# RustAudio/lewton

Measured on NVIDIA H100. Metric: Msamples/s IMDCT+window+OLA, 2048-pt long blocks, higher is better.
Workload: dtype f32

## Files before the change

lewton_b200/build.py:

```python
import os
import re
import shutil
import subprocess

HERE = os.path.dirname(os.path.abspath(__file__))
CSRC = os.path.join(HERE, "csrc")
SO = os.path.join(HERE, "liblewton_b200.so")
K_LONG_REGS = 249
SOURCES = ["lwb_api.cu", "host_objects.cuh", "path_generic.cuh", "path_long.cuh", "path_chain.cuh", "path_mixed.cuh", "path_mid.cuh",
           "tables_host.cpp", "frontend.cpp", "lwb_common.h", "pcm_copy_plan.h", "kernels_generic.cuh", "kernel_long.cuh", "kernel_deal.cuh", "kernel_short.cuh", "kernel_mid.cuh", "kernel_chain.cuh", "kernel_prologue.cuh", "kernel_floor0.cuh", "floor1_eval.cuh",
           "floor1_inverse_db.inc", "Makefile"]


def _stale():
    if not os.path.exists(SO):
        return True
    t = os.path.getmtime(SO)
    deps = [os.path.join(CSRC, s) for s in SOURCES] + [os.path.join(HERE, "..", "include", h)
                                                       for h in ("lewton_b200.h", "lewton_frontend.h")]
    return any(os.path.getmtime(d) > t for d in deps)


def check_no_fma(so=SO):
    if shutil.which("cuobjdump") is None:
        return None
    sass = subprocess.run(["cuobjdump", "-sass", so], capture_output=True, text=True, check=True).stdout
    bad = re.findall(r"^\s+/\*[0-9a-f]+\*/\s+(?:@!?U?P[0-9T]\s+)?(FFMA2?|DFMA)\b.*$", sass, re.M)
    return len(bad)


def hot_kernel_registers(log):
    regs = {}
    for m in re.finditer(r"Compiling entry function '(_ZN3lwb6k_longI([fs])EE[^']*)'.*?Used (\d+) registers", log, re.S):
        regs["k_long<float>" if m.group(2) == "f" else "k_long<int16_t>"] = int(m.group(3))
    return regs


def build(force=False, verbose=False):
    if force or _stale():
        if shutil.which("nvcc") is None:
            raise RuntimeError("nvcc not found: lewton_b200 has no CPU fallback and cannot be built without CUDA")
# ... 21 lines not shown
```

lewton_b200/csrc/kernel_long.cuh:

```cuda
#pragma once
#include <stdint.h>

#if defined(__CUDACC__)
#include <cuda_runtime.h>
#define LWB_HD __host__ __device__ __forceinline__
#else
#define LWB_HD inline
#endif

namespace lwb {

constexpr int kLongBs = 11;
constexpr int kLongN = 2048;
constexpr int kLongN2 = 1024;

struct alignas(16) LongRun {
    const float *in;
    void *out;
    float *state;
    uint32_t in_stride;
    uint32_t n_packets;
    uint8_t has_prev;
    uint8_t write_state;
    uint8_t dummy;
// ... 322 lines not shown
            const V b2 = vadd(O[b][d], O[b][e]);
            const V b3 = vsub(E[b][d], E[b][e]);
            O[b][d] = vadd(b2, b0);
            E[b][d] = vadd(b3, b1);
            O[b][e] = vsub(b2, b0);
            E[b][e] = vsub(b1, b3);
        }
    }
}

LWB_HD void step8_ola(V b0, V b1, V wlo, V whi, V Oj, V Ej, V prev_lo, V prev_hi, V &pcm_lo, V &pcm_hi, V &p_even)
{
    const V p_odd = vsub_p(vmul(Oj, b1), vmul(Ej, b0));
    p_even = vnsub_p(vmul(Oj, b0), vmul(Ej, b1));
    pcm_lo = vadd_p(vmul(p_odd, wlo), vmul(prev_lo, whi));
    pcm_hi = vsub_p(vmul(prev_hi, wlo), vmul(p_odd, whi));
}

#if defined(__CUDACC__)
#ifndef LWB_LONG_NB
#define LWB_LONG_NB 1
#endif
#ifndef LWB_LONG_WARPS
#define LWB_LONG_WARPS 8
#endif
#ifndef LWB_LONG_RING
#define LWB_LONG_RING (LWB_LONG_NB == 2 ? 2 : 5)
#endif
constexpr int kLongNB = LWB_LONG_NB;
constexpr int kLongWarps = LWB_LONG_WARPS;
constexpr int kLongRing = LWB_LONG_RING;
constexpr int kLongTileBytes = kLongN2 * 4;
constexpr int kLongStageBytes = kLongNB * kLongTileBytes;
constexpr size_t kLongSmemBytes = 2048 + (size_t)kLongWarps * (kLongRing + 1) * kLongStageBytes +
                                  (size_t)kLongPackFloats * 4 + kLongWarps * (kLongRing + 2) * 8 +
                                  kLongWarps * kLongNB * sizeof(LongRun) + 64;

__device__ __forceinline__ uint32_t smem_u32(const void *p) { return (uint32_t)__cvta_generic_to_shared(p); }

__device__ __forceinline__ void mbar_init(uint32_t bar, uint32_t count)
{
    asm volatile("mbarrier.init.shared::cta.b64 [%0], %1;" ::"r"(bar), "r"(count));
}
__device__ __forceinline__ void mbar_expect_tx(uint32_t bar, uint32_t bytes)
{
    asm volatile("mbarrier.arrive.expect_tx.shared::cta.b64 _, [%0], %1;" ::"r"(bar), "r"(bytes) : "memory");
}
__device__ __forceinline__ void mbar_wait(uint32_t bar, uint32_t parity)
{
    asm volatile(
        "{\n\t.reg .pred p;\n\t"
        "WAIT_%=:\n\t"
        "mbarrier.try_wait.parity.shared::cta.b64 p, [%0], %1, %2;\n\t"
        "@p bra DONE_%=;\n\t"
        "bra WAIT_%=;\n\t"
        "DONE_%=:\n\t}" ::"r"(bar), "r"(parity), "r"(200000u) : "memory");
}
__device__ __forceinline__ void tma_load_1d(uint32_t dst, const void *src, uint32_t bytes, uint32_t bar)
{
    asm volatile("cp.async.bulk.shared::cluster.global.mbarrier::complete_tx::bytes [%0], [%1], %2, [%3];"
                 ::"r"(dst), "l"(src), "r"(bytes), "r"(bar) : "memory");
}
__device__ __forceinline__ void fence_proxy_async()
{
    asm volatile("fence.proxy.async.shared::cta;" ::: "memory");
}
__device__ __forceinline__ void sts_eo(uint32_t addr, float e, float o)
{
    asm volatile("st.shared.f32 [%0], %1;\n\tst.shared.f32 [%0+2048], %2;" ::"r"(addr), "f"(e), "f"(o) : "memory");
}
__device__ __forceinline__ void lds_eo(uint32_t addr, float &e, float &o)
{
    asm volatile("ld.shared.f32 %0, [%2];\n\tld.shared.f32 %1, [%2+2048];" : "=f"(e), "=f"(o) : "r"(addr) : "memory");
}

}
#include "kernel_deal.cuh"
namespace lwb {

#ifndef LWB_TW_REG0
#define LWB_TW_REG0 0
#endif
#ifndef LWB_TW_REG1
#define LWB_TW_REG1 (LWB_LONG_NB == 2 ? 0 : 53)
#endif
constexpr int kTwReg0 = LWB_TW_REG0;
constexpr int kTwReg1 = LWB_TW_REG1;
struct TwMix {
    const V *r;
    const V *lane_base;
    __device__ __forceinline__ V operator()(int slot) const
    {
        return (slot >= kTwReg0 && slot < kTwReg1) ? r[slot - kTwReg0] : lane_base[slot * 32];
    }
};
// ... 6 lines not shown
#define LWB_KC(j) (4u * (uint32_t)swz(j))

struct RunCur {
    const float *in;
    void *out;
    float *state;
    uint32_t in_stride;
    uint32_t flags;
};
__device__ __forceinline__ RunCur run_cur(const LongRun &r)
{
    return RunCur{r.in, r.out, r.state, r.in_stride,
                  (uint32_t)(r.has_prev ? 1u : 0u) | (r.write_state ? 2u : 0u) | (r.dummy ? 4u : 0u) |
                      (r.first_short ? 8u : 0u) | (r.last_short ? 16u : 0u)};
}
struct RunCurS : RunCur { float *state_out; };
__device__ __forceinline__ RunCurS run_cur_s(const LongRun &r)
{
    RunCurS c;
    static_cast<RunCur &>(c) = run_cur(r);
    c.flags |= r.first_short == 2 ? 32u : 0u;
    c.state_out = r.state_out ? r.state_out : r.state;
    return c;
}

__device__ __forceinline__ int16_t d_sample_i16(float v)
{
    short r;
    asm("cvt.rzi.s16.f32 %0, %1;" : "=h"(r) : "f"(__fmul_rn(v, 32768.0f)));
    return (int16_t)r;
}
__device__ __forceinline__ void st_pcm(float *p, float v) { __stcs(p, v); }
__device__ __forceinline__ void st_pcm(int16_t *p, float v) { __stcs(reinterpret_cast<short *>(p), (short)d_sample_i16(v)); }

template <int NB, bool FIRST, typename OutT, typename RC = RunCur>
__device__ __forceinline__ void out_stage(const TwMix &tw, int lane, const V O[NB][8], const V E[NB][8], V pe[NB][8],
                                          const RC cur[NB], OutT *out[NB], const float *s_state)
{
#pragma unroll
    for (int j = 0; j < 8; j++) {
        const int r64 = 64 * rev3(j);
        const bool nat = (j & 1);
        const V b0 = tw(P_B0 + j), b1 = tw(P_B1 + j);
        const V wlo = tw(P_WLO + j), whi = tw(P_WHI + j);
#pragma unroll
        for (int b = 0; b < NB; b++) {
            V plo = pe[b][j], phi = pe[b][j];
            bool emit = !(cur[b].flags & 4u);
            if (FIRST) {
                emit = emit && (cur[b].flags & 1u);
                if (cur[b].flags & 1u) {
                    const float *s_lo = s_state + b * kLongN2 + lane, *s_hi = s_state + b * kLongN2 + 63 - lane;
                    const float ax = nat ? s_lo[r64] : s_hi[r64], ay = nat ? s_hi[r64] : s_lo[r64];
                    const float bx = nat ? s_hi[960 - r64] : s_lo[960 - r64];
                    const float by = nat ? s_lo[960 - r64] : s_hi[960 - r64];
                    plo = V{ax, ay};
                    phi = V{bx, by};
                }
            }
            V lo, hi, pev;
            step8_ola(b0, b1, wlo, whi, O[b][j], E[b][j], plo, phi, lo, hi, pev);
            pe[b][j] = pev;
            if (emit) {
                OutT *o_lo = out[b] + lane, *o_hi = out[b] + 63 - lane;
                if (nat) {
                    st_pcm(o_lo + r64, lo.x); st_pcm(o_hi + r64, lo.y);
                    st_pcm(o_hi + 960 - r64, hi.x); st_pcm(o_lo + 960 - r64, hi.y);
                } else {
                    st_pcm(o_hi + r64, lo.x); st_pcm(o_lo + r64, lo.y);
                    st_pcm(o_lo + 960 - r64, hi.x); st_pcm(o_hi + 960 - r64, hi.y);
                }
            }
        }
    }
}

__device__ __forceinline__ float lds_f32(uint32_t addr)
{
    float v;
    asm volatile("ld.shared.f32 %0, [%1];" : "=f"(v) : "r"(addr) : "memory");
    return v;
}

template <int NB, typename OutT, typename RC = RunCur, bool EXPORT = false, int LS = 0>
__device__ __forceinline__ void out_first_short(const TwMix &tw, int lane, const V O[NB][8], const V E[NB][8], V pe[NB][8],
                                                const RC cur[NB], OutT *out[NB], const float *s_state,
                                                const float *__restrict__ w, int ls_arg, uint32_t w_s = 0)
{
    const int ls = LS ? LS : ls_arg;
    const int pl = kLongN2 - 2 * ls;
#pragma unroll
    for (int j = 0; j < 8; j++) {
        const int r64 = 64 * rev3(j);
        const bool nat = (j & 1);
        const V b0 = tw(P_B0 + j), b1 = tw(P_B1 + j);
#pragma unroll
// ... 9 lines not shown
                const int m = r64 + ((h == 0) == nat ? lane : 63 - lane);
                static_assert(LS % 64 == 0, "LS must be a multiple of 64");
                const bool on_slope = LS ? (r64 >= LS) : (m >= ls);
                if (on_slope) {
                    const int i = m - ls;
                    const float cw = __fmul_rn(po, (EXPORT ? lds_f32(w_s + 4u * (uint32_t)i) : __ldg(w + i)));
                    if (exported) cur[b].state[i] = cw;
                    else st_pcm(out[b] + i, __fadd_rn(cw, __fmul_rn(prev[i], (EXPORT ? lds_f32(w_s + 4u * (uint32_t)(pl - 1 - i)) : __ldg(w + pl - 1 - i)))));
                }
                const int i = kLongN2 - 1 - m - ls;
                float v = -po;
                if (LS ? on_slope : (i < pl)) {
                    v = __fmul_rn(v, (EXPORT ? lds_f32(w_s + 4u * (uint32_t)i) : __ldg(w + i)));
                    if (exported) { cur[b].state[i] = v; continue; }
                    v = __fadd_rn(v, __fmul_rn(prev[i], (EXPORT ? lds_f32(w_s + 4u * (uint32_t)(pl - 1 - i)) : __ldg(w + pl - 1 - i))));
                }
                st_pcm(out[b] + i, v);
            }
        }
    }
}

template <typename OutT>
__global__ void __launch_bounds__(kLongWarps * 32, 1)
k_long(const LongRun *__restrict__ runs, uint32_t n_groups, const float *__restrict__ pack,
       unsigned int *__restrict__ ticket, const float *__restrict__ w_short, int ls)
{
    constexpr int NB = kLongNB;
    extern __shared__ __align__(128) unsigned char smem_raw[];
    const int lane = threadIdx.x & 31, warp = threadIdx.x >> 5;
    const uint32_t raw_s = smem_u32(smem_raw);
    const uint32_t align_pad = (2048u - (raw_s & 2047u)) & 2047u;
    unsigned char *base = smem_raw + align_pad;
    constexpr size_t kTilesBytes = (size_t)kLongWarps * kLongRing * kLongStageBytes;
    constexpr size_t kStateBytes = (size_t)kLongWarps * kLongStageBytes;
    float *tiles = reinterpret_cast<float *>(base) + (size_t)warp * kLongRing * NB * kLongN2;
    float *s_state = reinterpret_cast<float *>(base + kTilesBytes) + (size_t)warp * NB * kLongN2;
    V *s_pack = reinterpret_cast<V *>(base + kTilesBytes + kStateBytes);
    unsigned char *tail = base + kTilesBytes + kStateBytes + (size_t)kLongPackFloats * 4;
    LongRun *s_next = reinterpret_cast<LongRun *>(tail) + warp * NB;
    uint64_t *bars = reinterpret_cast<uint64_t *>(tail + (size_t)kLongWarps * NB * sizeof(LongRun)) +
                     warp * (kLongRing + 2);
    if (n_groups == 0) return;

    {
        const float4 *src = reinterpret_cast<const float4 *>(pack);
        float4 *dst = reinterpret_cast<float4 *>(s_pack);
        for (int i = threadIdx.x; i < kLongPackFloats / 4; i += blockDim.x) dst[i] = __ldg(src + i);
    }
    if (lane == 0) {
        for (int i = 0; i < kLongRing + 2; i++) mbar_init(smem_u32(&bars[i]), 1);
        asm volatile("fence.mbarrier_init.release.cluster;" ::: "memory");
    }
    __syncthreads();

    V twR[kTwReg1 - kTwReg0 > 0 ? kTwReg1 - kTwReg0 : 1];
#pragma unroll
    for (int s = kTwReg0; s < kTwReg1; s++) twR[s - kTwReg0] = s_pack[s * 32 + lane];
    const TwMix tw{twR, s_pack + lane};

    const uint32_t tiles_s = smem_u32(tiles);
    const uint32_t bars_s = smem_u32(bars);
    const uint32_t bar_state = bars_s + 8 * kLongRing, bar_desc = bars_s + 8 * (kLongRing + 1);
    const uint32_t state_s = smem_u32(s_state), next_s = smem_u32(s_next);
    const uint32_t lA0 = laneA(lane, 0), lA1 = laneA(lane, 1);
    const uint32_t lB = laneB(lane);
    const uint32_t lC0 = laneC(lane, 0), lC1 = laneC(lane, 1);
    uint32_t phase_bits = 0;
    uint32_t slot_i = 0;

    uint32_t lc = 0;
    uint32_t nx_idx = 0;
    uint32_t nx_stage = 0;
    uint32_t nx_lc = 0, nx_npk = 0;
    uint32_t nx_state_issued = 0;
    uint32_t desc_parity = 0;
    RunCur cur[NB];
    uint32_t npk;

    auto issue_stage = [&](uint32_t stage, const LongRun *r, uint32_t pkt) {
        const uint32_t bar = bars_s + 8 * stage;
        mbar_expect_tx(bar, kLongStageBytes);
#pragma unroll
        for (int b = 0; b < NB; b++)
            tma_load_1d(tiles_s + stage * kLongStageBytes + b * kLongTileBytes,
                        r[b].in + (size_t)pkt * r[b].in_stride, kLongTileBytes, bar);
    };
    auto issue_stage_cur = [&](uint32_t stage, uint32_t pkt) {
        const uint32_t bar = bars_s + 8 * stage;
        mbar_expect_tx(bar, kLongStageBytes);
#pragma unroll
        for (int b = 0; b < NB; b++)
            tma_load_1d(tiles_s + stage * kLongStageBytes + b * kLongTileBytes,
                        cur[b].in + (size_t)pkt * cur[b].in_stride, kLongTileBytes, bar);
    };
    auto issue_state = [&](const float *const st[NB], const uint32_t has[NB]) {
        uint32_t bytes = 0;
#pragma unroll
        for (int b = 0; b < NB; b++) bytes += has[b] ? kLongTileBytes : 0;
        mbar_expect_tx(bar_state, bytes);
#pragma unroll
        for (int b = 0; b < NB; b++)
            if (has[b]) tma_load_1d(state_s + b * kLongTileBytes, st[b], kLongTileBytes, bar_state);
    };

    {
        uint32_t idx = 0;
        if (lane == 0) idx = atomicAdd(ticket, 1u);
        idx = __shfl_sync(0xffffffffu, idx, 0);
        if (idx >= n_groups) return;
#pragma unroll
        for (int b = 0; b < NB; b++) cur[b] = run_cur(runs[idx * NB + b]);
        npk = runs[idx * NB].n_packets;
        if (lane == 0) {
            fence_proxy_async();
            const float *st[NB];
            uint32_t has[NB];
#pragma unroll
            for (int b = 0; b < NB; b++) { st[b] = cur[b].state; has[b] = cur[b].flags & 1u; }
            issue_state(st, has);
            for (; lc < (uint32_t)kLongRing && lc < npk; lc++) issue_stage_cur(lc, lc);
            nx_idx = atomicAdd(ticket, 1u);
        }
    }

    for (;;) {
        V pe[NB][8];
#pragma unroll
        for (int b = 0; b < NB; b++)
#pragma unroll
            for (int j = 0; j < 8; j++) pe[b][j] = V{0.f, 0.f};
        OutT *out[NB];
#pragma unroll
        for (int b = 0; b < NB; b++) out[b] = static_cast<OutT *>(cur[b].out);

        for (uint32_t p = 0; p < npk; p++) {
            const uint32_t stage_s = tiles_s + slot_i * kLongStageBytes;
            mbar_wait(bars_s + 8 * slot_i, (phase_bits >> slot_i) & 1u);
            phase_bits ^= 1u << slot_i;

            V O[NB][8], E[NB][8];
            {
                const float *tp[NB];
#pragma unroll
                for (int b = 0; b < NB; b++) tp[b] = tiles + (slot_i * NB + b) * kLongN2;
                phase_a<NB>(tp, lane, tw, O, E);
            }
            __syncwarp();
#pragma unroll
            for (int b = 0; b < NB; b++) {
                const uint32_t t = stage_s + b * kLongTileBytes;
                const uint32_t a0 = t + lA0, a1 = t + lA1;
#pragma unroll
                for (int j = 0; j < 8; j++) {
// ... 16 lines not shown
#pragma unroll
            for (int b = 0; b < NB; b++) {
                const uint32_t b0 = stage_s + b * kLongTileBytes + lB;
#pragma unroll
                for (int j = 0; j < 8; j++) {
                    sts_eo(b0 ^ LWB_KB(j, 0), E[b][j].x, O[b][j].x);
                    sts_eo(b0 ^ LWB_KB(j, 1), E[b][j].y, O[b][j].y);
                }
            }
            __syncwarp();
#pragma unroll
            for (int b = 0; b < NB; b++) {
                const uint32_t t = stage_s + b * kLongTileBytes;
                const uint32_t c0 = t + lC0, c1 = t + lC1;
#pragma unroll
                for (int j = 0; j < 8; j++) {
                    lds_eo(c0 ^ LWB_KC(j), E[b][j].x, O[b][j].x);
                    lds_eo(c1 ^ LWB_KC(j), E[b][j].y, O[b][j].y);
                }
            }
            __syncwarp();
            if (lane == 0) {
                if (nx_stage == 0 && p >= 1) {
                    if (nx_idx < n_groups) {
                        fence_proxy_async();
                        mbar_expect_tx(bar_desc, NB * (uint32_t)sizeof(LongRun));
                        tma_load_1d(next_s, runs + (size_t)nx_idx * NB, NB * (uint32_t)sizeof(LongRun), bar_desc);
                        nx_stage = 1;
                    } else {
                        nx_stage = 3;
                    }
                }
                uint32_t ahead = lc - (p + 1) + nx_lc;
                if (ahead < (uint32_t)kLongRing) {
                    uint32_t tgt = slot_i + 1 + ahead;
                    if (tgt >= (uint32_t)kLongRing) tgt -= kLongRing;
                    if (lc < npk) {
                        fence_proxy_async();
                        issue_stage_cur(tgt, lc);
                        lc++;
                    } else {
                        if (nx_stage == 1) {
                            mbar_wait(bar_desc, desc_parity);
                            desc_parity ^= 1u;
                            nx_stage = 2;
                            nx_npk = s_next[0].n_packets;
                            nx_lc = 0;
                        }
                        if (nx_stage == 2 && nx_lc < nx_npk) {
                            fence_proxy_async();
                            issue_stage(tgt, s_next, nx_lc);
                            nx_lc++;
                        }
                    }
                }
            }
            phase_c_fft<NB>(tw, O, E);
            if (p > 0) {
                out_stage<NB, false, OutT>(tw, lane, O, E, pe, cur, out, s_state);
            } else {
                mbar_wait(bar_state, (phase_bits >> 30) & 1u);
                phase_bits ^= 1u << 30;
                if (NB == 1 && (cur[0].flags & 8u))
                    out_first_short<NB, OutT>(tw, lane, O, E, pe, cur, out, s_state, w_short, ls);
                else
                    out_stage<NB, true, OutT>(tw, lane, O, E, pe, cur, out, s_state);
                __syncwarp();
            }
#pragma unroll
            for (int b = 0; b < NB; b++)
                if (p > 0 || (cur[b].flags & 1u)) out[b] += (p == 0 && (cur[b].flags & 8u)) ? kLongN2 - ls : kLongN2;
            if (lane == 0 && nx_stage == 2 && !nx_state_issued) {
                const float *st[NB];
                uint32_t has[NB];
#pragma unroll
                for (int b = 0; b < NB; b++) { st[b] = s_next[b].state; has[b] = s_next[b].has_prev; }
                fence_proxy_async();
                issue_state(st, has);
                nx_state_issued = 1;
            }
            slot_i = (slot_i + 1 == (uint32_t)kLongRing) ? 0 : slot_i + 1;
        }
#pragma unroll
        for (int b = 0; b < NB; b++) {
            if ((cur[b].flags & 16u)) {
                const bool emitted = (npk > 1 || (cur[b].flags & 1u)) && !(cur[b].flags & 4u);
                const bool keep = (cur[b].flags & 6u) == 2u;
#pragma unroll
                for (int j = 0; j < 8; j++) {
                    const int r64 = 64 * rev3(j);
#pragma unroll
                    for (int h = 0; h < 2; h++) {
                        const float v = ((j & 1) != 0) == (h == 0) ? pe[b][j].x : pe[b][j].y;
                        const int m = r64 + (h ? 63 - lane : lane);
                        if (m < ls) {
                            if (emitted) st_pcm(out[b] + m, v);
                        } else if (keep && m < kLongN2 - ls) {
                            cur[b].state[m - ls] = v;
                            cur[b].state[kLongN2 - 1 - ls - m] = v;
                        }
                    }
                }
            } else if ((cur[b].flags & 6u) == 2u) {
                float *s_lo = cur[b].state + lane, *s_hi = cur[b].state + 63 - lane;
#pragma unroll
                for (int j = 0; j < 8; j++) {
                    const int r64 = 64 * rev3(j);
                    const float vx = (j & 1) ? pe[b][j].x : pe[b][j].y, vy = (j & 1) ? pe[b][j].y : pe[b][j].x;
                    s_lo[r64] = vx; s_hi[r64] = vy;
                    s_hi[960 - r64] = vx; s_lo[960 - r64] = vy;
                }
            }
        }
        uint32_t st_ = 0, nlc = 0;
        if (lane == 0) {
            if (nx_stage == 0) {
                if (nx_idx < n_groups) {
                    fence_proxy_async();
                    mbar_expect_tx(bar_desc, NB * (uint32_t)sizeof(LongRun));
                    tma_load_1d(next_s, runs + (size_t)nx_idx * NB, NB * (uint32_t)sizeof(LongRun), bar_desc);
                    nx_stage = 1;
                } else {
                    nx_stage = 3;
                }
            }
            if (nx_stage == 1) {
                mbar_wait(bar_desc, desc_parity);
                desc_parity ^= 1u;
                nx_stage = 2;
                nx_npk = s_next[0].n_packets;
                nx_lc = 0;
            }
            if (nx_stage == 2 && !nx_state_issued) {
                const float *st[NB];
                uint32_t has[NB];
#pragma unroll
                for (int b = 0; b < NB; b++) { st[b] = s_next[b].state; has[b] = s_next[b].has_prev; }
                fence_proxy_async();
                issue_state(st, has);
            }
            st_ = nx_stage;
            nlc = nx_lc;
        }
        st_ = __shfl_sync(0xffffffffu, st_, 0);
        nlc = __shfl_sync(0xffffffffu, nlc, 0);
        if (st_ != 2) break;
        __syncwarp();
#pragma unroll
        for (int b = 0; b < NB; b++) cur[b] = run_cur(s_next[b]);
        npk = s_next[0].n_packets;
        __syncwarp();
        lc = nlc;
        nx_stage = 0; nx_lc = 0; nx_npk = 0; nx_state_issued = 0;
        if (lane == 0) {
            fence_proxy_async();
            for (uint32_t k = lc; k < (uint32_t)kLongRing && k < npk; k++) {
                issue_stage_cur((slot_i + k) % kLongRing, k);
                lc = k + 1;
            }
            nx_idx = atomicAdd(ticket, 1u);
        }
    }
}

constexpr int kLongLs256 = (kLongN - 256) / 4;
constexpr int kLongFetch = 3;
constexpr int kLongDescSlots = kLongFetch + kLongRing + 3;
constexpr int kLongSlopeMax = 512;
constexpr size_t kLongSmemBytesS = 2048 + (size_t)kLongWarps * (kLongRing + 1) * kLongTileBytes + (size_t)kLongPackFloats * 4 +
                                   kLongWarps * (kLongRing + 2) * 8 + (size_t)kLongWarps * kLongDescSlots * sizeof(LongRun) +
                                   kLongSlopeMax * sizeof(float) + 64;

__device__ __forceinline__ void transpose_abc(const TwMix &tw, uint32_t stage_s, uint32_t lA0, uint32_t lA1, uint32_t lB,
                                              uint32_t lC0, uint32_t lC1, V O[1][8], V E[1][8])
{
    __syncwarp();
    {
        const uint32_t a0 = stage_s + lA0, a1 = stage_s + lA1;
#pragma unroll
        for (int j = 0; j < 8; j++) {
            sts_eo(a0 ^ LWB_KA(j), E[0][j].x, O[0][j].x);
            sts_eo(a1 ^ LWB_KA(j), E[0][j].y, O[0][j].y);
        }
    }
    __syncwarp();
    {
        const uint32_t b0 = stage_s + lB;
#pragma unroll
        for (int j = 0; j < 8; j++) {
            lds_eo(b0 ^ LWB_KB(j, 0), E[0][j].x, O[0][j].x);
            lds_eo(b0 ^ LWB_KB(j, 1), E[0][j].y, O[0][j].y);
        }
    }
    __syncwarp();
    phase_b<1>(tw, O, E);
// ... 195 lines not shown
```

profiles/microbench/io_skeleton.cu:

```cuda
#include <cuda_runtime.h>
#include <cstdio>
#include <cstdint>
#include <cstdlib>

__device__ __forceinline__ uint32_t smem_u32(const void *p) { return (uint32_t)__cvta_generic_to_shared(p); }
__device__ __forceinline__ void mbar_init(uint32_t bar, uint32_t c) { asm volatile("mbarrier.init.shared::cta.b64 [%0], %1;" ::"r"(bar), "r"(c)); }
__device__ __forceinline__ void mbar_expect_tx(uint32_t bar, uint32_t b) { asm volatile("mbarrier.arrive.expect_tx.shared::cta.b64 _, [%0], %1;" ::"r"(bar), "r"(b) : "memory"); }
__device__ __forceinline__ void mbar_wait(uint32_t bar, uint32_t parity)
{
    asm volatile("{\n\t.reg .pred p;\n\tW_%=:\n\tmbarrier.try_wait.parity.shared::cta.b64 p, [%0], %1;\n\t@p bra D_%=;\n\tbra W_%=;\n\tD_%=:\n\t}" ::"r"(bar), "r"(parity) : "memory");
}
__device__ __forceinline__ void tma_load_1d(uint32_t dst, const void *src, uint32_t bytes, uint32_t bar)
{
    asm volatile("cp.async.bulk.shared::cluster.global.mbarrier::complete_tx::bytes [%0], [%1], %2, [%3];" ::"r"(dst), "l"(src), "r"(bytes), "r"(bar) : "memory");
}

template <int MODE>
__global__ void __launch_bounds__(384, 1) k_io(const float *__restrict__ in, float *__restrict__ out, uint32_t n_chains,
                                               uint32_t packets, unsigned int *ticket)
{
    extern __shared__ __align__(128) unsigned char smem[];
    const int lane = threadIdx.x & 31, warp = threadIdx.x >> 5;
    float *tiles = reinterpret_cast<float *>(smem) + warp * 3 * 1024;
    uint64_t *bars = reinterpret_cast<uint64_t *>(smem + 12 * 3 * 4096) + warp * 3;
    if (lane == 0) { for (int i = 0; i < 3; i++) mbar_init(smem_u32(&bars[i]), 1); asm volatile("fence.mbarrier_init.release.cluster;" ::: "memory"); }
    __syncthreads();
    uint32_t phase = 0;
    for (;;) {
        uint32_t c = 0;
        if (lane == 0) c = atomicAdd(ticket, 1u);
        c = __shfl_sync(0xffffffffu, c, 0);
        if (c >= n_chains) break;
        const float *src = in + (size_t)(c >> 1) * packets * 2048 + (c & 1) * 1024;
        float *dst = out + (size_t)c * packets * 1024;
        if (lane == 0)
            for (uint32_t i = 0; i < 3 && i < packets; i++) {
                mbar_expect_tx(smem_u32(&bars[i]), 4096);
                tma_load_1d(smem_u32(tiles + i * 1024), src + (size_t)i * 2048, 4096, smem_u32(&bars[i]));
            }
        uint32_t s = 0;
        for (uint32_t p = 0; p < packets; p++) {
            mbar_wait(smem_u32(&bars[s]), (phase >> s) & 1u);
            phase ^= 1u << s;
            const float4 *t4 = reinterpret_cast<const float4 *>(tiles + s * 1024);
            float4 q[8];
#pragma unroll
            for (int m = 0; m < 4; m++) { q[m] = t4[lane + 64 * m]; q[4 + m] = t4[63 - lane + 64 * m]; }
            __syncwarp();
            if (lane == 0 && p + 3 < packets) {
                asm volatile("fence.proxy.async.shared::cta;" ::: "memory");
                mbar_expect_tx(smem_u32(&bars[s]), 4096);
                tma_load_1d(smem_u32(tiles + s * 1024), src + (size_t)(p + 3) * 2048, 4096, smem_u32(&bars[s]));
            }
            float *o = dst + (size_t)p * 1024;
            if (MODE == 0) {
                const float v[32] = {q[0].x, q[0].y, q[0].z, q[0].w, q[1].x, q[1].y, q[1].z, q[1].w, q[2].x, q[2].y, q[2].z, q[2].w,
                                     q[3].x, q[3].y, q[3].z, q[3].w, q[4].x, q[4].y, q[4].z, q[4].w, q[5].x, q[5].y, q[5].z, q[5].w,
                                     q[6].x, q[6].y, q[6].z, q[6].w, q[7].x, q[7].y, q[7].z, q[7].w};
#pragma unroll
                for (int j = 0; j < 8; j++) {
                    const int r64 = 64 * (((j & 1) << 2) | (j & 2) | ((j >> 2) & 1));
                    __stcs(o + lane + r64, v[4 * j]);
                    __stcs(o + 63 - lane + r64, v[4 * j + 1]);
                    __stcs(o + 63 - lane + 960 - r64, v[4 * j + 2]);
                    __stcs(o + lane + 960 - r64, v[4 * j + 3]);
                }
            } else {
                float4 *o4 = reinterpret_cast<float4 *>(o);
#pragma unroll
                for (int m = 0; m < 8; m++) __stcs(o4 + lane + 32 * m, q[m]);
            }
            s = (s + 1 == 3) ? 0 : s + 1;
        }
    }
}

int main(int argc, char **argv)
{
    const uint32_t streams = 4096, packets = 16, chains = streams * 2;
    const size_t n = (size_t)chains * packets * 1024;
    float *in, *out;
    unsigned int *ticket;
    cudaMalloc(&in, n * 4); cudaMalloc(&out, n * 4); cudaMalloc(&ticket, 4096);
    cudaMemset(in, 0, n * 4);
    const size_t smem = 12 * 3 * 4096 + 12 * 3 * 8 + 64;
    cudaFuncSetAttribute(k_io<0>, cudaFuncAttributeMaxDynamicSharedMemorySize, (int)smem);
    cudaFuncSetAttribute(k_io<1>, cudaFuncAttributeMaxDynamicSharedMemorySize, (int)smem);
    int sms = 0;
    cudaDeviceGetAttribute(&sms, cudaDevAttrMultiProcessorCount, 0);
    cudaEvent_t e0, e1; cudaEventCreate(&e0); cudaEventCreate(&e1);
    for (int mode = 0; mode < 2; mode++) {
        float best = 1e9f;
        for (int it = 0; it < 12; it++) {
            cudaMemset(ticket, 0, 4);
            cudaEventRecord(e0);
            if (mode == 0) k_io<0><<<sms, 384, smem>>>(in, out, chains, packets, ticket);
            else k_io<1><<<sms, 384, smem>>>(in, out, chains, packets, ticket);
            cudaEventRecord(e1); cudaEventSynchronize(e1);
            float ms; cudaEventElapsedTime(&ms, e0, e1);
            if (it >= 2 && ms < best) best = ms;
        }
        printf("mode %d (%s): best %.3f ms  -> %.1f GB/s (read+write), err=%s\n", mode, mode ? "STG.128 coalesced" : "k_long line order STG.32",
               best, 2.0 * n * 4 / best / 1e6, cudaGetErrorString(cudaGetLastError()));
    }
    float best = 1e9f;
    for (int it = 0; it < 8; it++) {
        cudaEventRecord(e0); cudaMemcpyAsync(out, in, n * 4, cudaMemcpyDeviceToDevice); cudaEventRecord(e1); cudaEventSynchronize(e1);
        float ms; cudaEventElapsedTime(&ms, e0, e1); if (it >= 2 && ms < best) best = ms;
    }
    printf("cudaMemcpy D2D: best %.3f ms -> %.1f GB/s\n", best, 2.0 * n * 4 / best / 1e6);
    return 0;
}
```

Baseline: 322,800.

## Stage k_long PCM and state output in shared memory and write via bulk async stores

Each warp now writes its output block to a shared-memory staging tile and issues a TMA bulk store (cp.async.bulk, evict_first hint for PCM) instead of scattered per-lane STG.32 streaming stores. The final state write-back goes through the same staging path. To free shared memory for the staging tiles, the input prefetch ring drops by one stage. This aims to cut the store instruction count and the uncoalesced write traffic, at the cost of a shallower load pipeline and extra bulk-group waits before each stage is reused.

Result: no change. 325,100 (median of 6 runs) (+0.7%).

```diff
diff --git a/lewton_b200/build.py b/lewton_b200/build.py
--- a/lewton_b200/build.py
+++ b/lewton_b200/build.py
@@ -6,7 +6,7 @@
 HERE = os.path.dirname(os.path.abspath(__file__))
 CSRC = os.path.join(HERE, "csrc")
 SO = os.path.join(HERE, "liblewton_b200.so")
-K_LONG_REGS = 249
+K_LONG_REGS = 244
 SOURCES = ["lwb_api.cu", "host_objects.cuh", "path_generic.cuh", "path_long.cuh", "path_chain.cuh", "path_mixed.cuh", "path_mid.cuh",
            "tables_host.cpp", "frontend.cpp", "lwb_common.h", "pcm_copy_plan.h", "kernels_generic.cuh", "kernel_long.cuh", "kernel_deal.cuh", "kernel_short.cuh", "kernel_mid.cuh", "kernel_chain.cuh", "kernel_prologue.cuh", "kernel_floor0.cuh", "floor1_eval.cuh",
            "floor1_inverse_db.inc", "Makefile"]
diff --git a/lewton_b200/csrc/kernel_long.cuh b/lewton_b200/csrc/kernel_long.cuh
--- a/lewton_b200/csrc/kernel_long.cuh
+++ b/lewton_b200/csrc/kernel_long.cuh
@@ -378,9 +378,11 @@
 constexpr int kLongRing = LWB_LONG_RING;
 constexpr int kLongTileBytes = kLongN2 * 4;
 constexpr int kLongStageBytes = kLongNB * kLongTileBytes;
-constexpr size_t kLongSmemBytes = 2048 + (size_t)kLongWarps * (kLongRing + 1) * kLongStageBytes +
-                                  (size_t)kLongPackFloats * 4 + kLongWarps * (kLongRing + 2) * 8 +
+constexpr int kLongRingK = kLongRing - 1;
+constexpr size_t kLongSmemBytes = 2048 + (size_t)kLongWarps * (kLongRingK + 2) * kLongStageBytes +
+                                  (size_t)kLongPackFloats * 4 + kLongWarps * (kLongRingK + 2) * 8 +
                                   kLongWarps * kLongNB * sizeof(LongRun) + 64;
+static_assert(kLongSmemBytes <= 227 * 1024, "k_long needs more than the 227 KB of shared memory a CTA can opt in to");
 
 __device__ __forceinline__ uint32_t smem_u32(const void *p) { return (uint32_t)__cvta_generic_to_shared(p); }
 
@@ -407,6 +409,20 @@
     asm volatile("cp.async.bulk.shared::cluster.global.mbarrier::complete_tx::bytes [%0], [%1], %2, [%3];"
                  ::"r"(dst), "l"(src), "r"(bytes), "r"(bar) : "memory");
 }
+__device__ __forceinline__ void bulk_store_1d(void *dst, uint32_t src, uint32_t bytes)
+{
+    asm volatile("cp.async.bulk.global.shared::cta.bulk_group [%0], [%1], %2;\n\tcp.async.bulk.commit_group;"
+                 ::"l"(dst), "r"(src), "r"(bytes) : "memory");
+}
+__device__ __forceinline__ void bulk_store_1d_stream(void *dst, uint32_t src, uint32_t bytes)
+{
+    asm volatile("{\n\t.reg .b64 pol;\n\t"
+                 "createpolicy.fractional.L2::evict_first.b64 pol, 1.0;\n\t"
+                 "cp.async.bulk.global.shared::cta.bulk_group.L2::cache_hint [%0], [%1], %2, pol;\n\t"
+                 "cp.async.bulk.commit_group;\n\t}" ::"l"(dst), "r"(src), "r"(bytes) : "memory");
+}
+__device__ __forceinline__ void bulk_wait_read() { asm volatile("cp.async.bulk.wait_group.read 0;" ::: "memory"); }
+__device__ __forceinline__ void bulk_wait_all() { asm volatile("cp.async.bulk.wait_group 0;" ::: "memory"); }
 __device__ __forceinline__ void fence_proxy_async()
 {
     asm volatile("fence.proxy.async.shared::cta;" ::: "memory");
@@ -479,10 +495,16 @@
 }
 __device__ __forceinline__ void st_pcm(float *p, float v) { __stcs(p, v); }
 __device__ __forceinline__ void st_pcm(int16_t *p, float v) { __stcs(reinterpret_cast<short *>(p), (short)d_sample_i16(v)); }
-
-template <int NB, bool FIRST, typename OutT, typename RC = RunCur>
+template <typename OutT>
+__device__ __forceinline__ void sts_pcm(uint32_t a, float v)
+{
+    if constexpr (sizeof(OutT) == 4) asm volatile("st.shared.f32 [%0], %1;" ::"r"(a), "f"(v) : "memory");
+    else asm volatile("st.shared.b16 [%0], %1;" ::"r"(a), "h"(d_sample_i16(v)) : "memory");
+}
+
+template <int NB, bool FIRST, typename OutT, typename RC = RunCur, bool STAGED = false>
 __device__ __forceinline__ void out_stage(const TwMix &tw, int lane, const V O[NB][8], const V E[NB][8], V pe[NB][8],
-                                          const RC cur[NB], OutT *out[NB], const float *s_state)
+                                          const RC cur[NB], OutT *out[NB], const float *s_state, uint32_t stage_s = 0)
 {
 #pragma unroll
     for (int j = 0; j < 8; j++) {
@@ -508,7 +530,17 @@
             V lo, hi, pev;
             step8_ola(b0, b1, wlo, whi, O[b][j], E[b][j], plo, phi, lo, hi, pev);
             pe[b][j] = pev;
-            if (emit) {
+            if (STAGED && emit) {
+                constexpr uint32_t es = sizeof(OutT);
+                const uint32_t o_lo = stage_s + b * kLongTileBytes + es * lane, o_hi = stage_s + b * kLongTileBytes + es * (63 - lane);
+                if (nat) {
+                    sts_pcm<OutT>(o_lo + es * r64, lo.x); sts_pcm<OutT>(o_hi + es * r64, lo.y);
+                    sts_pcm<OutT>(o_hi + es * (960 - r64), hi.x); sts_pcm<OutT>(o_lo + es * (960 - r64), hi.y);
+                } else {
+                    sts_pcm<OutT>(o_hi + es * r64, lo.x); sts_pcm<OutT>(o_lo + es * r64, lo.y);
+                    sts_pcm<OutT>(o_lo + es * (960 - r64), hi.x); sts_pcm<OutT>(o_hi + es * (960 - r64), hi.y);
+                }
+            } else if (emit) {
                 OutT *o_lo = out[b] + lane, *o_hi = out[b] + 63 - lane;
                 if (nat) {
                     st_pcm(o_lo + r64, lo.x); st_pcm(o_hi + r64, lo.y);
@@ -584,15 +616,16 @@
     const uint32_t raw_s = smem_u32(smem_raw);
     const uint32_t align_pad = (2048u - (raw_s & 2047u)) & 2047u;
     unsigned char *base = smem_raw + align_pad;
-    constexpr size_t kTilesBytes = (size_t)kLongWarps * kLongRing * kLongStageBytes;
+    constexpr size_t kTilesBytes = (size_t)kLongWarps * kLongRingK * kLongStageBytes;
     constexpr size_t kStateBytes = (size_t)kLongWarps * kLongStageBytes;
-    float *tiles = reinterpret_cast<float *>(base) + (size_t)warp * kLongRing * NB * kLongN2;
+    float *tiles = reinterpret_cast<float *>(base) + (size_t)warp * kLongRingK * NB * kLongN2;
     float *s_state = reinterpret_cast<float *>(base + kTilesBytes) + (size_t)warp * NB * kLongN2;
-    V *s_pack = reinterpret_cast<V *>(base + kTilesBytes + kStateBytes);
-    unsigned char *tail = base + kTilesBytes + kStateBytes + (size_t)kLongPackFloats * 4;
+    const uint32_t out_s = smem_u32(base + kTilesBytes + kStateBytes) + warp * kLongStageBytes;
+    V *s_pack = reinterpret_cast<V *>(base + kTilesBytes + 2 * kStateBytes);
+    unsigned char *tail = base + kTilesBytes + 2 * kStateBytes + (size_t)kLongPackFloats * 4;
     LongRun *s_next = reinterpret_cast<LongRun *>(tail) + warp * NB;
     uint64_t *bars = reinterpret_cast<uint64_t *>(tail + (size_t)kLongWarps * NB * sizeof(LongRun)) +
-                     warp * (kLongRing + 2);
+                     warp * (kLongRingK + 2);
     if (n_groups == 0) return;
 
     {
@@ -601,7 +634,7 @@
         for (int i = threadIdx.x; i < kLongPackFloats / 4; i += blockDim.x) dst[i] = __ldg(src + i);
     }
     if (lane == 0) {
-        for (int i = 0; i < kLongRing + 2; i++) mbar_init(smem_u32(&bars[i]), 1);
+        for (int i = 0; i < kLongRingK + 2; i++) mbar_init(smem_u32(&bars[i]), 1);
         asm volatile("fence.mbarrier_init.release.cluster;" ::: "memory");
     }
     __syncthreads();
@@ -613,7 +646,7 @@
 
     const uint32_t tiles_s = smem_u32(tiles);
     const uint32_t bars_s = smem_u32(bars);
-    const uint32_t bar_state = bars_s + 8 * kLongRing, bar_desc = bars_s + 8 * (kLongRing + 1);
+    const uint32_t bar_state = bars_s + 8 * kLongRingK, bar_desc = bars_s + 8 * (kLongRingK + 1);
     const uint32_t state_s = smem_u32(s_state), next_s = smem_u32(s_next);
     const uint32_t lA0 = laneA(lane, 0), lA1 = laneA(lane, 1);
     const uint32_t lB = laneB(lane);
@@ -630,6 +663,19 @@
     RunCur cur[NB];
     uint32_t npk;
 
+    auto stage_acquire = [&]() {
+        if (lane == 0) bulk_wait_read();
+        __syncwarp();
+    };
+    auto stage_send_pcm = [&](OutT *const o[NB], bool first) {
+        fence_proxy_async();
+        __syncwarp();
+        if (lane == 0)
+#pragma unroll
+            for (int b = 0; b < NB; b++)
+                if (!(cur[b].flags & 4u) && (!first || (cur[b].flags & 1u)))
+                    bulk_store_1d_stream(o[b], out_s + b * kLongTileBytes, kLongN2 * (uint32_t)sizeof(OutT));
+    };
     auto issue_stage = [&](uint32_t stage, const LongRun *r, uint32_t pkt) {
         const uint32_t bar = bars_s + 8 * stage;
         mbar_expect_tx(bar, kLongStageBytes);
@@ -671,7 +717,7 @@
 #pragma unroll
             for (int b = 0; b < NB; b++) { st[b] = cur[b].state; has[b] = cur[b].flags & 1u; }
             issue_state(st, has);
-            for (; lc < (uint32_t)kLongRing && lc < npk; lc++) issue_stage_cur(lc, lc);
+            for (; lc < (uint32_t)kLongRingK && lc < npk; lc++) issue_stage_cur(lc, lc);
             nx_idx = atomicAdd(ticket, 1u);
         }
     }
@@ -754,9 +800,9 @@
                     }
                 }
                 uint32_t ahead = lc - (p + 1) + nx_lc;
-                if (ahead < (uint32_t)kLongRing) {
+                if (ahead < (uint32_t)kLongRingK) {
                     uint32_t tgt = slot_i + 1 + ahead;
-                    if (tgt >= (uint32_t)kLongRing) tgt -= kLongRing;
+                    if (tgt >= (uint32_t)kLongRingK) tgt -= kLongRingK;
                     if (lc < npk) {
                         fence_proxy_async();
                         issue_stage_cur(tgt, lc);
@@ -778,15 +824,29 @@
                 }
             }
             phase_c_fft<NB>(tw, O, E);
+            bool staged = true;
+#pragma unroll
+            for (int b = 0; b < NB; b++) staged = staged && !(reinterpret_cast<uintptr_t>(out[b]) & 15);
             if (p > 0) {
-                out_stage<NB, false, OutT>(tw, lane, O, E, pe, cur, out, s_state);
+                if (staged) {
+                    stage_acquire();
+                    out_stage<NB, false, OutT, RunCur, true>(tw, lane, O, E, pe, cur, out, s_state, out_s);
+                    stage_send_pcm(out, false);
+                } else {
+                    out_stage<NB, false, OutT>(tw, lane, O, E, pe, cur, out, s_state);
+                }
             } else {
                 mbar_wait(bar_state, (phase_bits >> 30) & 1u);
                 phase_bits ^= 1u << 30;
-                if (NB == 1 && (cur[0].flags & 8u))
+                if (NB == 1 && (cur[0].flags & 8u)) {
                     out_first_short<NB, OutT>(tw, lane, O, E, pe, cur, out, s_state, w_short, ls);
-                else
+                } else if (staged) {
+                    stage_acquire();
+                    out_stage<NB, true, OutT, RunCur, true>(tw, lane, O, E, pe, cur, out, s_state, out_s);
+                    stage_send_pcm(out, true);
+                } else {
                     out_stage<NB, true, OutT>(tw, lane, O, E, pe, cur, out, s_state);
+                }
                 __syncwarp();
             }
 #pragma unroll
@@ -801,7 +861,7 @@
                 issue_state(st, has);
                 nx_state_issued = 1;
             }
-            slot_i = (slot_i + 1 == (uint32_t)kLongRing) ? 0 : slot_i + 1;
+            slot_i = (slot_i + 1 == (uint32_t)kLongRingK) ? 0 : slot_i + 1;
         }
 #pragma unroll
         for (int b = 0; b < NB; b++) {
@@ -824,14 +884,18 @@
                     }
                 }
             } else if ((cur[b].flags & 6u) == 2u) {
-                float *s_lo = cur[b].state + lane, *s_hi = cur[b].state + 63 - lane;
+                stage_acquire();
+                const uint32_t s_lo = out_s + b * kLongTileBytes + 4u * lane, s_hi = out_s + b * kLongTileBytes + 4u * (63 - lane);
 #pragma unroll
                 for (int j = 0; j < 8; j++) {
-                    const int r64 = 64 * rev3(j);
+                    const uint32_t r64 = 64 * rev3(j);
                     const float vx = (j & 1) ? pe[b][j].x : pe[b][j].y, vy = (j & 1) ? pe[b][j].y : pe[b][j].x;
-                    s_lo[r64] = vx; s_hi[r64] = vy;
-                    s_hi[960 - r64] = vx; s_lo[960 - r64] = vy;
-                }
+                    sts_pcm<float>(s_lo + 4u * r64, vx); sts_pcm<float>(s_hi + 4u * r64, vy);
+                    sts_pcm<float>(s_hi + 4u * (960 - r64), vx); sts_pcm<float>(s_lo + 4u * (960 - r64), vy);
+                }
+                fence_proxy_async();
+                __syncwarp();
+                if (lane == 0) bulk_store_1d(cur[b].state, out_s + b * kLongTileBytes, kLongTileBytes);
             }
         }
         uint32_t st_ = 0, nlc = 0;
@@ -876,13 +940,14 @@
         nx_stage = 0; nx_lc = 0; nx_npk = 0; nx_state_issued = 0;
         if (lane == 0) {
             fence_proxy_async();
-            for (uint32_t k = lc; k < (uint32_t)kLongRing && k < npk; k++) {
-                issue_stage_cur((slot_i + k) % kLongRing, k);
+            for (uint32_t k = lc; k < (uint32_t)kLongRingK && k < npk; k++) {
+                issue_stage_cur((slot_i + k) % kLongRingK, k);
                 lc = k + 1;
             }
             nx_idx = atomicAdd(ticket, 1u);
         }
     }
+    if (lane == 0) bulk_wait_all();
 }
 
 constexpr int kLongLs256 = (kLongN - 256) / 4;
diff --git a/profiles/microbench/io_skeleton.cu b/profiles/microbench/io_skeleton.cu
--- a/profiles/microbench/io_skeleton.cu
+++ b/profiles/microbench/io_skeleton.cu
@@ -1,113 +1,237 @@
 #include <cuda_runtime.h>
+#include <algorithm>
+#include <cstdint>
 #include <cstdio>
-#include <cstdint>
 #include <cstdlib>
+#include <vector>
+
+constexpr uint32_t kStreams = 4096, kPackets = 16, kChains = kStreams * 2, kN2 = 1024, kWarps = 8;
 
 __device__ __forceinline__ uint32_t smem_u32(const void *p) { return (uint32_t)__cvta_generic_to_shared(p); }
 __device__ __forceinline__ void mbar_init(uint32_t bar, uint32_t c) { asm volatile("mbarrier.init.shared::cta.b64 [%0], %1;" ::"r"(bar), "r"(c)); }
 __device__ __forceinline__ void mbar_expect_tx(uint32_t bar, uint32_t b) { asm volatile("mbarrier.arrive.expect_tx.shared::cta.b64 _, [%0], %1;" ::"r"(bar), "r"(b) : "memory"); }
 __device__ __forceinline__ void mbar_wait(uint32_t bar, uint32_t parity)
 {
-    asm volatile("{\n\t.reg .pred p;\n\tW_%=:\n\tmbarrier.try_wait.parity.shared::cta.b64 p, [%0], %1;\n\t@p bra D_%=;\n\tbra W_%=;\n\tD_%=:\n\t}" ::"r"(bar), "r"(parity) : "memory");
+    asm volatile("{\n\t.reg .pred p;\n\tW_%=:\n\tmbarrier.try_wait.parity.shared::cta.b64 p, [%0], %1, %2;\n\t@p bra D_%=;\n\tbra W_%=;\n\tD_%=:\n\t}"
+                 ::"r"(bar), "r"(parity), "r"(200000u) : "memory");
 }
 __device__ __forceinline__ void tma_load_1d(uint32_t dst, const void *src, uint32_t bytes, uint32_t bar)
 {
     asm volatile("cp.async.bulk.shared::cluster.global.mbarrier::complete_tx::bytes [%0], [%1], %2, [%3];" ::"r"(dst), "l"(src), "r"(bytes), "r"(bar) : "memory");
 }
-
-template <int MODE>
-__global__ void __launch_bounds__(384, 1) k_io(const float *__restrict__ in, float *__restrict__ out, uint32_t n_chains,
-                                               uint32_t packets, unsigned int *ticket)
-{
-    extern __shared__ __align__(128) unsigned char smem[];
+__device__ __forceinline__ void bulk_store(void *dst, uint32_t src, uint32_t bytes)
+{
+    asm volatile("cp.async.bulk.global.shared::cta.bulk_group [%0], [%1], %2;\n\tcp.async.bulk.commit_group;" ::"l"(dst), "r"(src), "r"(bytes) : "memory");
+}
+__device__ __forceinline__ void bulk_wait_read() { asm volatile("cp.async.bulk.wait_group.read 0;" ::: "memory"); }
+__device__ __forceinline__ void bulk_wait_all() { asm volatile("cp.async.bulk.wait_group 0;" ::: "memory"); }
+__device__ __forceinline__ void fence_proxy_async() { asm volatile("fence.proxy.async.shared::cta;" ::: "memory"); }
+__device__ __forceinline__ float lds(uint32_t a) { float v; asm volatile("ld.shared.f32 %0, [%1];" : "=f"(v) : "r"(a) : "memory"); return v; }
+__device__ __forceinline__ void sts(uint32_t a, float v) { asm volatile("st.shared.f32 [%0], %1;" ::"r"(a), "f"(v) : "memory"); }
+__device__ __forceinline__ int rev3(int j) { return ((j & 1) << 2) | (j & 2) | ((j >> 2) & 1); }
+
+template <int RING> constexpr size_t smem_bytes() { return 2048 + (size_t)kWarps * (RING + 2) * 4096 + kWarps * (RING + 1) * 8 + 64; }
+
+template <bool BULK>
+__device__ __forceinline__ void put_block(float *o, uint32_t stage, int lane, const float v[32])
+{
+#pragma unroll
+    for (int j = 0; j < 8; j++) {
+        const int r64 = 64 * rev3(j);
+        const int idx[4] = {lane + r64, 63 - lane + r64, 63 - lane + 960 - r64, lane + 960 - r64};
+#pragma unroll
+        for (int k = 0; k < 4; k++) {
+            if (BULK) sts(stage + 4u * idx[k], v[4 * j + k]);
+            else __stcs(o + idx[k], v[4 * j + k]);
+        }
+    }
+}
+
+template <int RING, bool BULK>
+__global__ void __launch_bounds__(kWarps * 32, 1) k_io(const float *__restrict__ in, float *__restrict__ out, float *__restrict__ state,
+                                                       unsigned int *ticket)
+{
+    extern __shared__ __align__(128) unsigned char smem_raw[];
     const int lane = threadIdx.x & 31, warp = threadIdx.x >> 5;
-    float *tiles = reinterpret_cast<float *>(smem) + warp * 3 * 1024;
-    uint64_t *bars = reinterpret_cast<uint64_t *>(smem + 12 * 3 * 4096) + warp * 3;
-    if (lane == 0) { for (int i = 0; i < 3; i++) mbar_init(smem_u32(&bars[i]), 1); asm volatile("fence.mbarrier_init.release.cluster;" ::: "memory"); }
-    __syncthreads();
-    uint32_t phase = 0;
+    const uint32_t raw_s = smem_u32(smem_raw);
+    unsigned char *base = smem_raw + ((2048u - (raw_s & 2047u)) & 2047u);
+    const uint32_t tiles_s = smem_u32(base) + warp * RING * 4096;
+    const uint32_t state_s = smem_u32(base) + kWarps * RING * 4096 + warp * 4096;
+    const uint32_t stage_s = smem_u32(base) + kWarps * (RING + 1) * 4096 + warp * 4096;
+    const float *tiles = reinterpret_cast<const float *>(base) + (size_t)warp * RING * kN2;
+    const uint32_t bars_s = smem_u32(base) + kWarps * (RING + 2) * 4096 + warp * (RING + 1) * 8, bar_state = bars_s + 8 * RING;
+    if (lane == 0) {
+        for (int i = 0; i <= RING; i++) mbar_init(bars_s + 8 * i, 1);
+        asm volatile("fence.mbarrier_init.release.cluster;" ::: "memory");
+    }
+    __syncwarp();
+    uint32_t nxt = 0;
+    if (lane == 0) nxt = atomicAdd(ticket, 1u);
+    uint32_t c = __shfl_sync(0xffffffffu, nxt, 0);
+    if (c >= kChains) return;
+    auto src_of = [&](uint32_t ch, uint32_t p) { return in + ((size_t)(ch >> 1) * kPackets * 2 + p * 2 + (ch & 1)) * kN2; };
+    if (lane == 0) {
+        mbar_expect_tx(bar_state, 4096);
+        tma_load_1d(state_s, state + (size_t)c * kN2, 4096, bar_state);
+        for (int i = 0; i < RING; i++) { mbar_expect_tx(bars_s + 8 * i, 4096); tma_load_1d(tiles_s + i * 4096, src_of(c, i), 4096, bars_s + 8 * i); }
+        nxt = atomicAdd(ticket, 1u);
+    }
+    uint32_t phase = 0, t = 0, k = 0;
     for (;;) {
-        uint32_t c = 0;
-        if (lane == 0) c = atomicAdd(ticket, 1u);
-        c = __shfl_sync(0xffffffffu, c, 0);
-        if (c >= n_chains) break;
-        const float *src = in + (size_t)(c >> 1) * packets * 2048 + (c & 1) * 1024;
-        float *dst = out + (size_t)c * packets * 1024;
-        if (lane == 0)
-            for (uint32_t i = 0; i < 3 && i < packets; i++) {
-                mbar_expect_tx(smem_u32(&bars[i]), 4096);
-                tma_load_1d(smem_u32(tiles + i * 1024), src + (size_t)i * 2048, 4096, smem_u32(&bars[i]));
-            }
-        uint32_t s = 0;
-        for (uint32_t p = 0; p < packets; p++) {
-            mbar_wait(smem_u32(&bars[s]), (phase >> s) & 1u);
+        float *dst = out + (size_t)c * kPackets * kN2;
+        float carry[32];
+        for (uint32_t p = 0; p < kPackets; p++, t++) {
+            const uint32_t s = t % RING;
+            mbar_wait(bars_s + 8 * s, (phase >> s) & 1u);
             phase ^= 1u << s;
-            const float4 *t4 = reinterpret_cast<const float4 *>(tiles + s * 1024);
-            float4 q[8];
-#pragma unroll
-            for (int m = 0; m < 4; m++) { q[m] = t4[lane + 64 * m]; q[4 + m] = t4[63 - lane + 64 * m]; }
+            const float4 *t4 = reinterpret_cast<const float4 *>(tiles + s * kN2);
+            float v[32];
+#pragma unroll
+            for (int m = 0; m < 4; m++) {
+                const float4 a = t4[lane + 64 * m], b = t4[63 - lane + 64 * m];
+                v[8 * m + 0] = a.x; v[8 * m + 1] = a.y; v[8 * m + 2] = a.z; v[8 * m + 3] = a.w;
+                v[8 * m + 4] = b.x; v[8 * m + 5] = b.y; v[8 * m + 6] = b.z; v[8 * m + 7] = b.w;
+            }
             __syncwarp();
-            if (lane == 0 && p + 3 < packets) {
-                asm volatile("fence.proxy.async.shared::cta;" ::: "memory");
-                mbar_expect_tx(smem_u32(&bars[s]), 4096);
-                tma_load_1d(smem_u32(tiles + s * 1024), src + (size_t)(p + 3) * 2048, 4096, smem_u32(&bars[s]));
-            }
-            float *o = dst + (size_t)p * 1024;
-            if (MODE == 0) {
-                const float v[32] = {q[0].x, q[0].y, q[0].z, q[0].w, q[1].x, q[1].y, q[1].z, q[1].w, q[2].x, q[2].y, q[2].z, q[2].w,
-                                     q[3].x, q[3].y, q[3].z, q[3].w, q[4].x, q[4].y, q[4].z, q[4].w, q[5].x, q[5].y, q[5].z, q[5].w,
-                                     q[6].x, q[6].y, q[6].z, q[6].w, q[7].x, q[7].y, q[7].z, q[7].w};
+            if (lane == 0) {
+                const uint32_t u = t + RING, ku = u / kPackets;
+                const uint32_t ch = ku == k ? c : nxt;
+                if (ch < kChains) {
+                    fence_proxy_async();
+                    mbar_expect_tx(bars_s + 8 * s, 4096);
+                    tma_load_1d(tiles_s + s * 4096, src_of(ch, u % kPackets), 4096, bars_s + 8 * s);
+                }
+            }
+            if (p == 0) {
+                mbar_wait(bar_state, (phase >> 30) & 1u);
+                phase ^= 1u << 30;
 #pragma unroll
                 for (int j = 0; j < 8; j++) {
-                    const int r64 = 64 * (((j & 1) << 2) | (j & 2) | ((j >> 2) & 1));
-                    __stcs(o + lane + r64, v[4 * j]);
-                    __stcs(o + 63 - lane + r64, v[4 * j + 1]);
-                    __stcs(o + 63 - lane + 960 - r64, v[4 * j + 2]);
-                    __stcs(o + lane + 960 - r64, v[4 * j + 3]);
+                    const int r64 = 64 * rev3(j);
+                    carry[4 * j + 0] = lds(state_s + 4u * (lane + r64));
+                    carry[4 * j + 1] = lds(state_s + 4u * (63 - lane + r64));
+                    carry[4 * j + 2] = lds(state_s + 4u * (63 - lane + 960 - r64));
+                    carry[4 * j + 3] = lds(state_s + 4u * (lane + 960 - r64));
                 }
+                __syncwarp();
+#pragma unroll
+                for (int i = 0; i < 32; i++) v[i] = __int_as_float(__float_as_int(v[i]) ^ __float_as_int(carry[i]));
+            } else if (p == 1 && lane == 0 && nxt < kChains) {
+                fence_proxy_async();
+                mbar_expect_tx(bar_state, 4096);
+                tma_load_1d(state_s, state + (size_t)nxt * kN2, 4096, bar_state);
+            }
+            if (BULK) {
+                if (lane == 0) bulk_wait_read();
+                __syncwarp();
+                put_block<true>(nullptr, stage_s, lane, v);
+                fence_proxy_async();
+                __syncwarp();
+                if (lane == 0) bulk_store(dst + (size_t)p * kN2, stage_s, 4096);
             } else {
-                float4 *o4 = reinterpret_cast<float4 *>(o);
-#pragma unroll
-                for (int m = 0; m < 8; m++) __stcs(o4 + lane + 32 * m, q[m]);
-            }
-            s = (s + 1 == 3) ? 0 : s + 1;
-        }
-    }
-}
-
-int main(int argc, char **argv)
-{
-    const uint32_t streams = 4096, packets = 16, chains = streams * 2;
-    const size_t n = (size_t)chains * packets * 1024;
-    float *in, *out;
+                put_block<false>(dst + (size_t)p * kN2, 0, lane, v);
+            }
+#pragma unroll
+            for (int i = 0; i < 32; i++) carry[i] = v[i];
+        }
+        float *st = state + (size_t)c * kN2;
+        if (BULK) {
+            if (lane == 0) bulk_wait_read();
+            __syncwarp();
+#pragma unroll
+            for (int j = 0; j < 8; j++) {
+                const int r64 = 64 * rev3(j);
+                sts(stage_s + 4u * (lane + r64), carry[4 * j]); sts(stage_s + 4u * (63 - lane + r64), carry[4 * j + 1]);
+                sts(stage_s + 4u * (63 - lane + 960 - r64), carry[4 * j]); sts(stage_s + 4u * (lane + 960 - r64), carry[4 * j + 1]);
+            }
+            fence_proxy_async();
+            __syncwarp();
+            if (lane == 0) bulk_store(st, stage_s, 4096);
+        } else {
+#pragma unroll
+            for (int j = 0; j < 8; j++) {
+                const int r64 = 64 * rev3(j);
+                st[lane + r64] = carry[4 * j]; st[63 - lane + r64] = carry[4 * j + 1];
+                st[63 - lane + 960 - r64] = carry[4 * j]; st[lane + 960 - r64] = carry[4 * j + 1];
+            }
+        }
+        k++;
+        c = __shfl_sync(0xffffffffu, nxt, 0);
+        if (c >= kChains) break;
+        if (lane == 0) nxt = atomicAdd(ticket, 1u);
+    }
+    if (BULK && lane == 0) bulk_wait_all();
+}
+
+__global__ void k_copy_f4(const float4 *__restrict__ in, float4 *__restrict__ out, size_t n4)
+{
+    for (size_t i = blockIdx.x * (size_t)blockDim.x + threadIdx.x; i < n4; i += (size_t)gridDim.x * blockDim.x) __stcs(out + i, __ldcs(in + i));
+}
+
+#define CK(x) do { cudaError_t e_ = (x); if (e_ != cudaSuccess) { fprintf(stderr, "%s: %s\n", #x, cudaGetErrorString(e_)); exit(1); } } while (0)
+
+int main()
+{
+    const size_t n = (size_t)kChains * kPackets * kN2;
+    float *in, *out, *state;
     unsigned int *ticket;
-    cudaMalloc(&in, n * 4); cudaMalloc(&out, n * 4); cudaMalloc(&ticket, 4096);
-    cudaMemset(in, 0, n * 4);
-    const size_t smem = 12 * 3 * 4096 + 12 * 3 * 8 + 64;
-    cudaFuncSetAttribute(k_io<0>, cudaFuncAttributeMaxDynamicSharedMemorySize, (int)smem);
-    cudaFuncSetAttribute(k_io<1>, cudaFuncAttributeMaxDynamicSharedMemorySize, (int)smem);
-    int sms = 0;
-    cudaDeviceGetAttribute(&sms, cudaDevAttrMultiProcessorCount, 0);
-    cudaEvent_t e0, e1; cudaEventCreate(&e0); cudaEventCreate(&e1);
-    for (int mode = 0; mode < 2; mode++) {
-        float best = 1e9f;
-        for (int it = 0; it < 12; it++) {
-            cudaMemset(ticket, 0, 4);
-            cudaEventRecord(e0);
-            if (mode == 0) k_io<0><<<sms, 384, smem>>>(in, out, chains, packets, ticket);
-            else k_io<1><<<sms, 384, smem>>>(in, out, chains, packets, ticket);
-            cudaEventRecord(e1); cudaEventSynchronize(e1);
-            float ms; cudaEventElapsedTime(&ms, e0, e1);
-            if (it >= 2 && ms < best) best = ms;
-        }
-        printf("mode %d (%s): best %.3f ms  -> %.1f GB/s (read+write), err=%s\n", mode, mode ? "STG.128 coalesced" : "k_long line order STG.32",
-               best, 2.0 * n * 4 / best / 1e6, cudaGetErrorString(cudaGetLastError()));
-    }
-    float best = 1e9f;
-    for (int it = 0; it < 8; it++) {
-        cudaEventRecord(e0); cudaMemcpyAsync(out, in, n * 4, cudaMemcpyDeviceToDevice); cudaEventRecord(e1); cudaEventSynchronize(e1);
-        float ms; cudaEventElapsedTime(&ms, e0, e1); if (it >= 2 && ms < best) best = ms;
-    }
-    printf("cudaMemcpy D2D: best %.3f ms -> %.1f GB/s\n", best, 2.0 * n * 4 / best / 1e6);
+    CK(cudaMalloc(&in, n * 4)); CK(cudaMalloc(&out, n * 4)); CK(cudaMalloc(&state, (size_t)kChains * kN2 * 4)); CK(cudaMalloc(&ticket, 4));
+    CK(cudaMemset(in, 0, n * 4)); CK(cudaMemset(state, 0, (size_t)kChains * kN2 * 4));
+    CK(cudaFuncSetAttribute(k_io<5, false>, cudaFuncAttributeMaxDynamicSharedMemorySize, (int)smem_bytes<5>()));
+    CK(cudaFuncSetAttribute(k_io<4, true>, cudaFuncAttributeMaxDynamicSharedMemorySize, (int)smem_bytes<4>()));
+    cudaDeviceProp prop;
+    CK(cudaGetDeviceProperties(&prop, 0));
+    {
+        char cmd[128], line[256] = "?";
+        snprintf(cmd, sizeof cmd, "nvidia-smi --query-gpu=power.limit,clocks.max.sm --format=csv,noheader -i %02x:%02x.0", prop.pciBusID, prop.pciDeviceID);
+        if (FILE *f = popen(cmd, "r")) { if (!fgets(line, sizeof line, f)) snprintf(line, sizeof line, "?\n"); pclose(f); }
+        printf("device: %s, %d SMs; power limit, max SM clock: %s", prop.name, prop.multiProcessorCount, line);
+    }
+    const int sms = prop.multiProcessorCount;
+    const double io_bytes = 2.0 * n * 4, run_bytes = io_bytes + 2.0 * kChains * kN2 * 4;
+    struct Var { const char *name; double bytes; int kind; };
+    const Var vars[] = {{"copy_d2d", io_bytes, 0}, {"copy_f4", io_bytes, 1}, {"stg_ring5", run_bytes, 2}, {"bulk_ring4", run_bytes, 3}};
+    auto launch = [&](int kind) {
+        switch (kind) {
+        case 0: CK(cudaMemcpyAsync(out, in, n * 4, cudaMemcpyDeviceToDevice)); break;
+        case 1: k_copy_f4<<<sms * 8, 512>>>(reinterpret_cast<const float4 *>(in), reinterpret_cast<float4 *>(out), n / 4); break;
+        case 2: CK(cudaMemsetAsync(ticket, 0, 4)); k_io<5, false><<<sms, kWarps * 32, smem_bytes<5>()>>>(in, out, state, ticket); break;
+        default: CK(cudaMemsetAsync(ticket, 0, 4)); k_io<4, true><<<sms, kWarps * 32, smem_bytes<4>()>>>(in, out, state, ticket); break;
+        }
+    };
+    cudaEvent_t e0, e1;
+    CK(cudaEventCreate(&e0)); CK(cudaEventCreate(&e1));
+    int reps[4];
+    for (int v = 0; v < 4; v++) {
+        for (int i = 0; i < 3; i++) launch(vars[v].kind);
+        CK(cudaEventRecord(e0));
+        for (int i = 0; i < 10; i++) launch(vars[v].kind);
+        CK(cudaEventRecord(e1)); CK(cudaEventSynchronize(e1)); CK(cudaGetLastError());
+        float ms; CK(cudaEventElapsedTime(&ms, e0, e1));
+        reps[v] = std::max(10, (int)(250.0f / (ms / 10)) + 1);
+    }
+    const int rounds = 6;
+    std::vector<double> gbs[4];
+    double secs[4] = {0, 0, 0, 0};
+    for (int r = 0; r < rounds; r++)
+        for (int v = 0; v < 4; v++) {
+            CK(cudaEventRecord(e0));
+            for (int i = 0; i < reps[v]; i++) launch(vars[v].kind);
+            CK(cudaEventRecord(e1)); CK(cudaEventSynchronize(e1)); CK(cudaGetLastError());
+            float ms; CK(cudaEventElapsedTime(&ms, e0, e1));
+            gbs[v].push_back(vars[v].bytes * reps[v] / (ms * 1e-3) / 1e9);
+            secs[v] += ms * 1e-3;
+        }
+    double med_of[4];
+    for (int v = 0; v < 4; v++) {
+        std::sort(gbs[v].begin(), gbs[v].end());
+        med_of[v] = 0.5 * (gbs[v][(rounds - 1) / 2] + gbs[v][rounds / 2]);
+    }
+    const double ceiling = std::max(med_of[0], med_of[1]);
+    for (int v = 0; v < 4; v++) {
+        const double med = med_of[v];
+        printf("%-11s %7.1f GB/s median over %d rounds (%.1f-%.1f), %.2f s in all, %.3f ms per launch, %.3f of the best copy, %.3f of 3350 GB/s\n",
+               vars[v].name, med, rounds, gbs[v].front(), gbs[v].back(), secs[v], vars[v].bytes / med / 1e6, med / ceiling, med / 3350.0);
+    }
     return 0;
 }
```
